# ultravideo/kvazaar

Measured on AMD Instinct MI355X. Metric: CTUs/s (all-intra ultrafast hot path), higher is better.
Workload: dtype u8/i16 (f64 RD costs); 1 GPU; 1920x1080 yuv420p 8-bit all-intra ultrafast CTU pass (kvz_hip_intra_frames), QP 22; ctus_per_frame=510, distinct_frames=8, wpp=True, parallelism=frames sharded over 1 GPU(s), no data-path collective

## Files before the change

### include/kvz_hip_dev.h

```cpp
#ifndef KVZ_HIP_DEV_H_
#define KVZ_HIP_DEV_H_

#include "kvz_hip_types.h"

#ifdef __cplusplus
extern "C" {
#endif

void *kvz_hip_dev_alloc(size_t bytes);
void  kvz_hip_dev_free(void *p);
void  kvz_hip_dev_upload(void *dev_dst, const void *host_src, size_t bytes);
void  kvz_hip_dev_download(void *host_dst, const void *dev_src, size_t bytes);
void  kvz_hip_dev_sync(void);
void  kvz_hip_dev_copy(void *dev_dst, const void *dev_src, size_t bytes);
void  kvz_hip_dev_timer_start(void);
float kvz_hip_dev_timer_stop(void);

int  kvz_hip_dev_sad_nxn(int n, const uint8_t *a, const uint8_t *b, int count, uint32_t *out);
int  kvz_hip_dev_satd_nxn(int n, const uint8_t *a, const uint8_t *b, int count, uint32_t *out);

int  kvz_hip_dev_transform(int kind, const int16_t *in, int16_t *tmp, int16_t *out, int count, int use_matrix_cores);

int  kvz_hip_dev_angular_pred(int log2_width, int mode, const uint8_t *ref_above, const uint8_t *ref_left, int count, uint8_t *out);

int  kvz_hip_dev_intra_select(int log2w, int nblk, const uint32_t *raw, const int8_t *preds, const double *mode_bits, int count, int32_t *winner);

int  kvz_hip_dev_cu8_units(int count, int from_coeffs, const int16_t *in, const int32_t *qp, int16_t *levels, int16_t *dequant, int16_t *resid);

int  kvz_hip_dev_satd8_blocks(const uint8_t *a, const uint8_t *b, int count, uint32_t *out);

int  kvz_hip_dev_rough_rows(int log2w, const uint8_t *top, const uint8_t *left, int count, uint8_t *out);

void kvz_hip_dev_deblock_frames(uint8_t *frames, int width, int height, int n_frames, const uint8_t *cu_depth, int qp, int beta_offset_div2,
                                int tc_offset_div2);

typedef struct kvz_hip_cu_dbk {
  uint8_t type;
  uint8_t depth, tr_depth, part_size;
  uint8_t cbf_y;
  uint8_t mv_dir;
  int8_t  mv_ref[2];
  int16_t ref_id[2];
  int16_t mv[2][2];
} kvz_hip_cu_dbk;
void kvz_hip_dev_deblock_frames_inter(uint8_t *frames, int width, int height, int n_frames, const kvz_hip_cu_dbk *info, int qp, int beta_offset_div2,
                                      int tc_offset_div2, int slice_is_b);
// ... 131 lines not shown
```

### kvazaar_amd/csrc/kvz_ctu.hpp

```cpp
#pragma once
#include <type_traits>
#include "../../include/kvz_hip_types.h"
#include "kvz_ops.hpp"
#include "kvz_rdoq.hpp"
#include "kvz_recon.hpp"
#include "kvz_residual.hpp"
#include "kvz_select.hpp"

namespace kvz {

#define KVZ_CTU_THREADS 128
#ifdef KVZ_HOSTSIM
#define KVZ_FOR_THREADS(tid) for (int tid = 0; tid < KVZ_CTU_THREADS; ++tid)
#ifdef KVZ_HOSTSIM_COUNT_SYNCS
static unsigned long long g_kvz_syncs;
#define KVZ_SYNC() (++g_kvz_syncs)
#else
#define KVZ_SYNC()
#endif
#define KVZ_LDS_ADD(p, v) (*(p) += (v))
#else
#define KVZ_FOR_THREADS(tid) for (int tid = (threadIdx.x + lane_rot) & (KVZ_CTU_THREADS - 1), once_ = 1; once_; once_ = 0)
#define KVZ_SYNC() __syncthreads()
#define KVZ_LDS_ADD(p, v) atomicAdd((p), (v))
// ... 62 lines not shown
  const unsigned t = __builtin_amdgcn_alignbit(x, x, 16);
  Pk16 sw, r;
  __builtin_memcpy(&sw, &t, 4);
  r = a * pk_make(1, -1) + sw;
  unsigned rr;
  __builtin_memcpy(&rr, &r, 4);
  return __builtin_amdgcn_sad_u16(rr, 0x80008000u, acc);
}
#define KVZ_PK_BIAS pk_make(-32768, 0)
#endif

#ifndef KVZ_HOSTSIM
}
#include "kvz_mfma.hpp"
namespace kvz {
#endif

#define KVZ_PROF_PU_AT (2 * KVZ_P_COUNT + 16)
#define KVZ_PROF_W32_AT (4 * KVZ_P_COUNT + 16)
#define KVZ_PROF_WORDS (6 * KVZ_P_COUNT + 16)
enum { KVZ_P_INIT = 0, KVZ_P_REFS, KVZ_P_PRED35, KVZ_P_SATD, KVZ_P_SELECT, KVZ_P_RPRED, KVZ_P_FDCT, KVZ_P_QUANT, KVZ_P_IDCT, KVZ_P_RECON,
       KVZ_P_COST, KVZ_P_COPY, KVZ_P_FINISH, KVZ_P_MISC, KVZ_P_COEFFBITS, KVZ_P_RDOQ, KVZ_P_COUNT };
#if defined(KVZ_CTU_PROFILE) && !defined(KVZ_HOSTSIM)
#define KVZ_PROF(cat) prof_mark(cat)
#define KVZ_PROF_SYNC(cat) do { KVZ_SYNC(); prof_mark(cat); } while (0)
#else
#define KVZ_PROF(cat)
#define KVZ_PROF_SYNC(cat)
#endif

// ... 750 lines not shown
        s->ref[c][side][k] = have ? base[off] : (u8)128;
        if (c) s->ref[2][side][k] = have ? base[off + dv] : (u8)128;
      }
    }
    KVZ_SYNC();
    KVZ_FOR_THREADS(tid) {
      if (luma) {
        const int n = 2 * (1 << log2w_y) + 1;
        for (int i = tid; i < 2 * n; i += KVZ_CTU_THREADS) {
          const int side = i >= n, k = side ? i - n : i;
          s->fref[side][k] = luma_filtered_ref(&s->ref[0][0][0], n, i);
        }
      }
      const int c = mover_lane(tid) - (KVZ_CTU_THREADS - 3);
      if (c >= 0 && ((c == 0 && luma) || (c > 0 && chroma))) {
        const int l2 = c ? log2w_c : log2w_y, w = 1 << l2;
#ifdef KVZ_HOSTSIM
        s->dcval[c] = (u8)dc_value(l2, s->ref[c][0], s->ref[c][1]);
#else
        u32 sum = 0;
        for (int i = 0; i < w; i += 4) {
          u32 a, b;
          __builtin_memcpy(&a, &s->ref[c][0][1 + i], 4);
          __builtin_memcpy(&b, &s->ref[c][1][1 + i], 4);
          sum = __builtin_amdgcn_sad_u8(a, 0u, sum);
          sum = __builtin_amdgcn_sad_u8(b, 0u, sum);
        }
        s->dcval[c] = (u8)((sum + w) >> (l2 + 1));
#endif
      }
    }
    KVZ_SYNC();
    KVZ_PROF(KVZ_P_REFS);
  }

  KVZ_DEV u8 predict_pixel(int log2w, int mode, int c, int x, int y) const
  {
    const int w = 1 << log2w;
    const u8 *top = s->ref[c][0], *left = s->ref[c][1];
    if (c == 0 && luma_reads_filtered(log2w, mode)) { top = s->fref[0]; left = s->fref[1]; }
    if (mode == 0) return planar_pixel(log2w, x, y, top, left);
    if (mode == 1) {
      const int dc = s->dcval[c];
// ... 26 lines not shown
      const u8 *pa = a + r * as, *pb = b + r * bs;
      int d[8];
      for (int x = 0; x < 8; x++) d[x] = (int)pa[x] - (int)pb[x];
      int u0, u1, u2, u3;
      if (col & 4) { u0 = d[0] - d[4]; u1 = d[1] - d[5]; u2 = d[2] - d[6]; u3 = d[3] - d[7]; }
      else { u0 = d[0] + d[4]; u1 = d[1] + d[5]; u2 = d[2] + d[6]; u3 = d[3] + d[7]; }
      const int v0 = (col & 2) ? u0 - u2 : u0 + u2, v1 = (col & 2) ? u1 - u3 : u1 + u3;
      t[r] = (col & 1) ? v0 - v1 : v0 + v1;
    }
    KVZ_HAD8(t[0], t[1], t[2], t[3], t[4], t[5], t[6], t[7]);
    u32 sum = 0;
    for (int r = 0; r < 8; r++) sum += (u32)iabs(t[r]);
    return sum;
  }

#ifndef KVZ_HOSTSIM
  KVZ_DEV static Pk16 as_pk16(U16x2 v) { Pk16 r; __builtin_memcpy(&r, &v, 4); return r; }
  KVZ_DEV static void widen8(const u8 *p, U16x2 out[4])
  {
    unsigned w[2];
    __builtin_memcpy(w, p, 8);
    out[0] = widen(0, w[0], 0x0c010c00u); out[1] = widen(0, w[0], 0x0c030c02u); out[2] = widen(0, w[1], 0x0c010c00u); out[3] = widen(0, w[1], 0x0c030c02u);
  }
#endif
  template <bool PAIR>
  KVZ_DEV u32 angular_block_satd(int log2w, int mode, int bx, int by, int xl, int yl, int half) const
  {
    const int w = 1 << log2w;
    const bool big = S32 && log2w == 5;
    const bool flat = mode < 2;
    const bool vertical = mode >= 18 || flat;
    const int disp = s->mode_disp[mode];
    const int p0 = vertical ? bx : by, q0 = vertical ? by : bx;
    const u8 *mr;
    if (disp < 0) mr = big ? mref32() + (mode - 11) * KVZ_MREF32_STRIDE + KVZ_MREF32_ORG : s->mref[mode - 11] + KVZ_MREF_ORG;
    else {
      const bool filt = imin(iabs(mode - 26), iabs(mode - 10)) > (log2w == 3 ? 7 : (log2w == 4 ? 1 : 0));
      mr = filt ? s->fref[vertical ? 0 : 1] : s->ref[0][vertical ? 0 : 1];
    }
// ... 81 lines not shown
#ifndef KVZ_HOSTSIM
      return sum;
#endif
    }
    return 2 * sum;
  }

#ifndef KVZ_HOSTSIM
  KVZ_DEV u32 angular_group_satd(const SatdWalsh &wm, const dev_int4 rows[2], const dev_int4 o[2]) const
  {
    dev_int4 p[2];
    satd_rows_predict(&s->ref[0][0][0], rows, p);
    return satd8_group_mfma(wm, p, o);
  }

  KVZ_DEV u32 flat_block_satd8(int log2w, int mode, int bx, int by, int xl, int yl, int lane) const
  {
    const int w = 1 << log2w, r = lane & 7, y = by + r;
    U16x2 o[4], v[4];
    widen8(org_at(0, xl + bx, yl + y), o);
    if (mode == 0) {
      const u8 *top = s->fref[0], *left = s->fref[1];
      const int tr = top[w + 1], bl = left[w + 1], l = left[y + 1];
      U16x2 tp[4];
      widen8(top + bx + 1, tp);
      const U16x2 dl = splat16(tr - l), wy = splat16(w - 1 - y), hb = splat16((w - 1) * l + tr + (y + 1) * bl + w);
#pragma unroll
      for (int j = 0; j < 4; j++) {
        U16x2 xs;
        xs.x = (unsigned short)(bx + 2 * j); xs.y = (unsigned short)(bx + 2 * j + 1);
        v[j] = (xs * dl + (tp[j] * wy + hb)) >> (unsigned short)(log2w + 1);
      }
    } else if (mode == 1) {
      const u8 *top = s->ref[0][0], *left = s->ref[0][1];
      const int dc = s->dcval[0];
      U16x2 tp[4];
      widen8(top + bx + 1, tp);
#pragma unroll
      for (int j = 0; j < 4; j++) v[j] = y == 0 ? (U16x2)((tp[j] + splat16(3 * dc + 2)) >> (unsigned short)2) : splat16(dc);
      if (bx == 0) v[0].x = (unsigned short)(y == 0 ? (left[1] + 2 * dc + top[1] + 2) >> 2 : (left[y + 1] + 3 * dc + 2) >> 2);
    } else {
      widen8(s->fref[0] + bx + y + 2, v);
    }
    Pk16 d[4];
#pragma unroll
    for (int j = 0; j < 4; j++) d[j] = as_pk16(v[j] - o[j]);
    if (r == 0) d[0] = pk_add(d[0], KVZ_PK_BIAS);
    {
      const Pk16 a0 = pk_add(d[0], d[2]), a1 = pk_add(d[1], d[3]), a2 = pk_sub(d[0], d[2]), a3 = pk_sub(d[1], d[3]);
      d[0] = pk_add(a0, a1); d[1] = pk_sub(a0, a1); d[2] = pk_add(a2, a3); d[3] = pk_sub(a2, a3);
    }
#define KVZ_FLAT8_STAGE(ctrl, bit)                                                                          \
    {                                                                                                       \
      const Pk16 sgn = pk_make((lane & (bit)) ? -1 : 1, (lane & (bit)) ? -1 : 1);                           \
      _Pragma("unroll") for (int j = 0; j < 4; j++) {                                                       \
        int mine;                                                                                           \
        __builtin_memcpy(&mine, &d[j], 4);                                                                  \
        const int theirs = __builtin_amdgcn_update_dpp(0, mine, ctrl, 0xF, 0xF, true);                       \
        Pk16 ot;                                                                                            \
        __builtin_memcpy(&ot, &theirs, 4);                                                                  \
        d[j] = ot * sgn + d[j];                                                                             \
      }                                                                                                     \
    }
    KVZ_FLAT8_STAGE(0x141 , 4)
    KVZ_FLAT8_STAGE(0x4E , 2)
    KVZ_FLAT8_STAGE(0xB1 , 1)
#undef KVZ_FLAT8_STAGE
    u32 sum = pk_abs2_biased(d[3], pk_abs2_biased(d[2], pk_abs2_biased(d[1], pk_abs2_biased(d[0], 0))));
    sum += (u32)__builtin_amdgcn_update_dpp(0, (int)sum, 0xB1, 0xF, 0xF, true);
    sum += (u32)__builtin_amdgcn_update_dpp(0, (int)sum, 0x4E, 0xF, 0xF, true);
    sum += (u32)__builtin_amdgcn_update_dpp(0, (int)sum, 0x141, 0xF, 0xF, true);
    return sum;
  }
#endif

  template <int L2>
  KVZ_DEV void build_mref(int tid, const u32 *pre = nullptr)
  {
    constexpr int W = 1 << L2, NQ = 2 * W + 2, N = (15 * NQ + KVZ_CTU_THREADS - 1) / KVZ_CTU_THREADS;
    u8 vals[N];
    if constexpr (L2 != 5) {
      static_assert(N * KVZ_CTU_THREADS <= 512, "Tables::mref_tab rows");
      u32 e[N];
      for (int k = 0; k < N; k++) e[k] = pre ? pre[k] : tb->mref_tab[L2 - 3][tid + k * KVZ_CTU_THREADS];
      mref_copy<N>(&s->ref[0][0][0], e);
      return;
    }
    for (int k = 0; k < N; k++) {
// ... 77 lines not shown
  {
    const int log2w = 6 - depth, w = 1 << log2w, xl = x - cx, yl = y - cy, nblk = (w >> 3) * (w >> 3);
#ifndef KVZ_HOSTSIM
    u32 mref_pre[4] = { 0, 0, 0, 0 };
    if (!(S32 && log2w == 5)) {
      const u32 *row = tb->mref_tab[log2w - 3] + ((threadIdx.x + lane_rot) & (KVZ_CTU_THREADS - 1));
      for (int k = 0; k < 4; k++) mref_pre[k] = row[k * KVZ_CTU_THREADS];
    }
    dev_int4 rows_pre[2][2] = {};
    {
      const int t = (threadIdx.x + lane_rot) & (KVZ_CTU_THREADS - 1);
      if (log2w == 4 || (log2w == 3 && t < 64)) {
        const dev_int4 *row = reinterpret_cast<const dev_int4 *>(tb->satd_rows[log2w == 4 ? 1 + 2 * (t >> 6) : 0][t & 63]);
        rows_pre[0][0] = row[0]; rows_pre[0][1] = row[1];
        if (log2w == 4) { rows_pre[1][0] = row[2 * 64]; rows_pre[1][1] = row[2 * 64 + 1]; }
      }
    }
#endif
    build_refs(lv, x, y, log2w, depth == 3 ? 2 : log2w - 1, true, true, first);
    if (S32 && log2w == 5) {
      KVZ_FOR_THREADS(tid) {
        if constexpr (S32) build_mref<5>(tid);
        u8 *ot = org_t32();
        for (int e = tid; e < 1024; e += KVZ_CTU_THREADS) ot[e] = *org_at(0, xl + (e >> 5), yl + (e & 31));
        for (int v = tid; v < 35; v += KVZ_CTU_THREADS) s->satd_raw[v][0] = 0;
        if (tid == KVZ_CTU_THREADS - 1) {
          int left, above;
          neighbour_pair(lv, x, y, &left, &above);
          mpm_candidates(y, left, above, s->preds);
        }
// ... 48 lines not shown
      }
#else
      if (log2w == 4 || tid < 64) {
        const int lane = tid & 63;
        const SatdWalsh wm = satd8_walsh(tb, lane);
        dev_int4 o[2];
        satd_rows_source(&s->ref[0][0][0], org_at(0, xl, yl), rows_pre[0], o);
        const int p = (log2w == 4 ? 64 * (tid >> 6) : 0) + (lane & 31), mode = 2 + (p >> lb), b = p & (nblk - 1);
        const u32 v0 = angular_group_satd(wm, rows_pre[0], o);
        if (lane < 32) s->satd_raw[mode][b] = v0;
        if (log2w == 4) {
          const u32 v1 = angular_group_satd(wm, rows_pre[1], o);
          if (lane < 32) s->satd_raw[mode + 8][b] = v1;
        }
      }
      {
        const int t = KVZ_CTU_THREADS - 1 - tid;
        if (t < 24 * nblk) {
          const int mb = t >> 3, mi = mb >> lb, mode = mi == 0 ? 34 : mi - 1, b = mb & (nblk - 1), bx = (b & ((w >> 3) - 1)) * 8, by = (b >> (log2w - 3)) * 8;
          const u32 v = flat_block_satd8(log2w, mode, bx, by, xl, yl, tid);
          if ((tid & 7) == 0) s->satd_raw[mode][b] = v;
        }
      }
#endif
    }
    }
    KVZ_SYNC();
    KVZ_PROF(KVZ_P_SATD);
    KVZ_FOR_THREADS(tid) {
      if (tid >= kHookThread && tid < kHookThread + kCostEntries) cu_cost_prepare(lv, x, y, depth, tid - kHookThread);
      const int final_mode = replay_selection(tid, log2w, nblk);
      if (final_mode >= 0) {
        if (tid == 0) s->best_mode = final_mode;
#ifdef KVZ_HOSTSIM
        const int holders = 1;
#else
// ... 1839 lines not shown
```

### kvazaar_amd/csrc/kvz_dev.hpp

```cpp
#pragma once
#include <hip/hip_runtime.h>

#include <functional>
#include <mutex>
#include <chrono>
#include <vector>

#include "../../include/kvz_hip_dev.h"
#include "kvz_mfma.hpp"
#include "kvz_ops.hpp"
#include "kvz_sao.hpp"
#include "kvz_entropy.hpp"
#include "kvz_select.hpp"
#include "kvz_recon.hpp"
#include "kvz_tables.hpp"

namespace kvz {

__device__ __forceinline__ u32 load_u32_any(const u8 *p) { u32 v; __builtin_memcpy(&v, p, 4); return v; }
template <int G> __device__ __forceinline__ u32 group_sum(u32 v)
{
  for (int off = G / 2; off > 0; off >>= 1) v += __shfl_down(v, off, G);
  return v;
}
// ... 317 lines not shown
    const int g = L2 == 4 ? 2 * (tid >> 6) + j : 0, pr = 32 * g + (lane & 31), mode = 2 + (pr >> LB), b = pr & (NBLK - 1);
    const dev_int4 *row = reinterpret_cast<const dev_int4 *>(tb->satd_rows[L2 == 4 ? 1 + g : 0][lane]);
    const dev_int4 e[2] = { row[0], row[1] };
    dev_int4 p[2];
    satd_rows_predict(ref0, e, p);
    u8 *o = out + ((cu * 32 + (mode - 2)) * NBLK + b) * 64;
#pragma unroll
    for (int i = 0; i < 4; i++)
#pragma unroll
      for (int x = 0; x < 8; x++) {
        const int r = 4 * (lane >> 5) + i;
        const u8 v = (u8)(((u32)p[i >> 1][2 * (i & 1) + (x >> 2)] >> (8 * (x & 3))) ^ 0x80);
        o[mode >= 18 ? 8 * r + x : 8 * x + r] = v;
      }
  }
}

template <int L2> __global__ void __launch_bounds__(256) dev_angular_kernel(const u8 *above, const u8 *left, const int count, const int mode, u8 *out)
{
  constexpr int W = 1 << L2, NG = kAngularGroupsPerLane, GPB = W * W / 4, BLOCKS = 256 * NG / GPB, RS = 2 * W + 1, ES = (2 * W + 1 + 8 + 3) & ~3;
  constexpr int RAW = (BLOCKS * RS + 3 + 3) / 4 + 2;
  __shared__ u32 s_raw[2][RAW];
  __shared__ alignas(8) u8 s_ext[BLOCKS][ES];
  __shared__ u32 s_tile[BLOCKS * W * W / 4];
  const int disp_tab[9] = { 0, 2, 5, 9, 13, 17, 21, 26, 32 };
  const int inv_tab[9] = { 0, 4096, 1638, 910, 630, 482, 390, 315, 256 };
  const bool vertical = mode >= 18;
  const int mode_disp = vertical ? mode - 26 : 10 - mode, ad = iabs(mode_disp);
  const int disp = mode_disp < 0 ? -disp_tab[ad] : disp_tab[ad], inv = inv_tab[ad];
  const long blk0 = (long)blockIdx.x * BLOCKS;
// ... 873 lines not shown
}

int kvz_hip_dev_cu8_units(int count, int from_coeffs, const int16_t *in, const int32_t *qp, int16_t *levels, int16_t *dequant, int16_t *resid)
{
  if (count < 0 || (from_coeffs != 0 && from_coeffs != 1)) { fprintf(stderr, "kvz_hip_dev_cu8_units: count=%d from_coeffs=%d\n", count, from_coeffs); return -1; }
  if (count == 0) return 0;
  KVZ_DEV_LAUNCH(kvz::dev_cu8_units_kernel, ((long)count + 1) / 2 * 256, in, qp, count, from_coeffs, kvz::device_tables(), levels, dequant, resid);
  return 0;
}

int kvz_hip_dev_rough_rows(int log2w, const uint8_t *top, const uint8_t *left, int count, uint8_t *out)
{
  if (count < 0 || (log2w != 3 && log2w != 4)) { fprintf(stderr, "kvz_hip_dev_rough_rows: log2w=%d count=%d\n", log2w, count); return -1; }
  if (log2w == 3) KVZ_DEV_LAUNCH(kvz::dev_rough_rows_kernel<3>, ((long)count + 1) / 2 * 256, kvz::device_tables(), top, left, count, out);
  else KVZ_DEV_LAUNCH(kvz::dev_rough_rows_kernel<4>, ((long)count + 1) / 2 * 256, kvz::device_tables(), top, left, count, out);
  return 0;
}

int kvz_hip_dev_satd8_blocks(const uint8_t *a, const uint8_t *b, int count, uint32_t *out)
{
  if (count < 0) { fprintf(stderr, "kvz_hip_dev_satd8_blocks: count=%d\n", count); return -1; }
  KVZ_DEV_LAUNCH(kvz::dev_satd8_blocks_kernel, ((long)count + 31) / 32 * 64, kvz::device_tables(), a, b, count, out);
  return 0;
}

void kvz_hip_dev_deblock_frames(uint8_t *frames, int width, int height, int n_frames, const uint8_t *cu_depth, int qp, int beta_offset_div2,
                                int tc_offset_div2)
{
  kvz::deblock_frames_on(be().stream, frames, width, height, n_frames, cu_depth, qp, beta_offset_div2, tc_offset_div2);
}
// ... 1035 lines not shown
```

### kvazaar_amd/csrc/kvz_mfma.hpp

```cpp
#pragma once
#include <hip/hip_runtime.h>

#include "kvz_ops.hpp"

namespace kvz {

typedef int dev_int4 __attribute__((ext_vector_type(4)));
typedef int dev_int16 __attribute__((ext_vector_type(16)));

__device__ __forceinline__ void dev_byte_planes(int v0, int v1, int v2, int v3, u32 &lo, u32 &hi)
{
  const u32 t01 = __builtin_amdgcn_perm((u32)v1, (u32)v0, 0x05010400u), t23 = __builtin_amdgcn_perm((u32)v3, (u32)v2, 0x05010400u);
  lo = __builtin_amdgcn_perm(t23, t01, 0x05040100u) ^ 0x80808080u;
  hi = __builtin_amdgcn_perm(t23, t01, 0x07060302u);
}

template <int N> struct DevMma;
template <> struct DevMma<16> {
  static constexpr int NREG = 4;
  static __device__ __forceinline__ int idx(int lane) { return lane & 15; }
  static __device__ __forceinline__ int row(int lane, int r) { return 4 * (lane >> 4) + r; }
  static __device__ __forceinline__ int k0(int lane, int) { return 4 * (lane >> 4); }
  static constexpr int STEPS = 1;
};
// ... 181 lines not shown
  }
}
__device__ __forceinline__ void satd_rows_source(const u8 *ref0, const u8 *cu_org, const dev_int4 e[2], dev_int4 o[2])
{
  const u8 *base = ((unsigned)e[0][1] >> 16 & kSatdSrcVertical) ? cu_org : ref0;
#pragma unroll
  for (int i = 0; i < 4; i++) {
    const unsigned src = (unsigned)e[i >> 1][2 * (i & 1) + 1] >> 16 & (kSatdSrcVertical - 1);
    unsigned ow[2];
    __builtin_memcpy(ow, __builtin_assume_aligned(base + src, 8), 8);
    o[i >> 1][2 * (i & 1)] = (int)(ow[0] ^ 0x80808080u);
    o[i >> 1][2 * (i & 1) + 1] = (int)(ow[1] ^ 0x80808080u);
  }
}

__device__ __forceinline__ void dev_satd8_blocks_wave(const Tables *tb, const u8 *a, const u8 *bsrc, int count, u32 *out, int group, int lane)
{
  const long blk = 32l * group + (lane & 31);
  const bool live = blk < count;
  dev_int4 p[2] = {}, o[2] = {};
  if (live) {
    const dev_int4 *pa = reinterpret_cast<const dev_int4 *>(a + 64 * blk + 32 * (lane >> 5)), *po = reinterpret_cast<const dev_int4 *>(bsrc + 64 * blk + 32 * (lane >> 5));
    p[0] = pa[0]; p[1] = pa[1]; o[0] = po[0]; o[1] = po[1];
  }
#pragma unroll
  for (int q = 0; q < 2; q++) { p[q] ^= (int)0x80808080u; o[q] ^= (int)0x80808080u; }
  const u32 v = satd8_group_mfma(satd8_walsh(tb, lane), p, o);
  if (live && lane < 32) out[blk] = v;
}

// ... 2 lines not shown
```

### kvazaar_amd/csrc/kvz_ops.hpp

```cpp
#pragma once
#include <stdint.h>

#ifdef KVZ_HOSTSIM
#define KVZ_DEV inline
#define KVZ_ATOMIC_ADD(p, v) (*(p) += (v))
#else
#include <hip/hip_runtime.h>
#define KVZ_DEV __device__ __forceinline__
#define KVZ_ATOMIC_ADD(p, v) atomicAdd((p), (v))
#endif

namespace kvz {

typedef uint8_t u8;
typedef int16_t i16;
typedef uint16_t u16;
typedef uint32_t u32;
typedef int32_t i32;

#ifdef KVZ_HOSTSIM
#define KVZ_HD inline
#else
#define KVZ_HD __host__ __device__ __forceinline__
#endif
// ... 34 lines not shown
  alignas(16) i32 dct_sum[2][2][32];
  alignas(16) int8_t bd_i8[3][2][16 * 16];
  alignas(16) i32 bd_sum[3][2][16];
  u32 small_pairs[3][2][8][4];
  u32 pairs16[2][16][8];
  u32 scan[3][4][1024];
  u8 avail_top[16][16], avail_left[16][16];
  u8 ctx_next[2][128];
  u32 mref_tab[2][512];
  u8 diag8[64];
  u32 entropy_bits[128];
  int8_t luma_filter[4][8];
  int8_t chroma_filter[8][4];
  alignas(16) u32 satd_walsh[64][8];
  alignas(16) u32 satd_rows[5][64][8];
};

struct SatdRow { unsigned window, edge, src; int df; bool vertical; };
KVZ_HD SatdRow satd_row_of(u32 w0, u32 w1)
{
  SatdRow r;
  r.window = w0 & 0xffff; r.edge = w0 >> 16; r.df = (int)(w1 & 0xffff) >> 3; r.vertical = (w1 >> 16 & kSatdSrcVertical) != 0; r.src = w1 >> 16 & (kSatdSrcVertical - 1);
  return r;
}
KVZ_HD void satd_row_walk(const u8 *ref0, u32 w0, u32 w1, u8 out[8])
{
  const SatdRow r = satd_row_of(w0, w1);
  const u8 *m = ref0 + r.window;
  for (int k = 0; k < 8; k++) out[k] = (u8)(((32 - r.df) * m[k] + r.df * m[k + 1] + 16) >> 5);
  out[0] ^= ref0[r.edge];
}
KVZ_HD u8 satd_edge_byte(const u8 *ref0, int log2w, int i)
{
  const int o = i >> log2w, q = i & ((1 << log2w) - 1);
  const u8 *side = ref0 + kMrefRefRow * (1 - o);
  const int main1 = ref0[kMrefRefRow * o + 1];
  return (u8)(iclip(0, 255, main1 + (((int)side[q + 1] - (int)side[0]) >> 1)) ^ main1);
}
template <int N> KVZ_DEV void mref_copy(u8 *ref0, const u32 e[N])
{
  u8 vals[N];
  for (int k = 0; k < N; k++) vals[k] = ref0[e[k] & 0xffff];
  for (int k = 0; k < N; k++) ref0[kMrefExtended + (e[k] >> 16)] = vals[k];
}
KVZ_HD u8 luma_filtered_ref(const u8 *ref0, int n, int i)
{
  const int side = i >= n, k = side ? i - n : i;
  const u8 *r = ref0 + kMrefRefRow * side;
  if (k == 0) return (u8)((ref0[kMrefRefRow + 1] + 2 * ref0[kMrefRefRow] + ref0[1] + 2) / 4);
  if (k == n - 1) return r[k];
  return (u8)((r[k - 1] + 2 * r[k] + r[k + 1] + 2) / 4);
}
// ... 417 lines not shown
{
  const int w = 1 << log2w;
  const int hor = (w - 1 - x) * left[y + 1] + (x + 1) * top[w + 1];
  const int ver = (w - 1 - y) * top[x + 1] + (y + 1) * left[w + 1];
  return (u8)((ver + hor + w) >> (log2w + 1));
}

KVZ_DEV int dc_value(int log2w, const u8 *top, const u8 *left)
{
  const int w = 1 << log2w;
  int sum = 0;
  for (int i = 0; i < w; i++) sum += top[i + 1] + left[i + 1];
  return (u8)((sum + w) >> (log2w + 1));
}

KVZ_DEV u8 filtered_dc_pixel(int dc, int x, int y, const u8 *top, const u8 *left)
{
  if (x == 0 && y == 0) return (u8)((left[1] + 2 * dc + top[1] + 2) / 4);
  if (y == 0) return (u8)((top[x + 1] + 3 * dc + 2) / 4);
  if (x == 0) return (u8)((left[y + 1] + 3 * dc + 2) / 4);
  return (u8)dc;
}

struct IntraPredOp {
  int kind, log2w; const int8_t *modes ; const u8 *above; const u8 *left; long ref_bstride; u8 *dst;
  KVZ_DEV void operator()(int item) const
  {
    const int w = 1 << log2w, blk = item >> (2 * log2w), e = item & (w * w - 1), y = e >> log2w, x = e & (w - 1);
    const u8 *t = above + blk * ref_bstride, *l = left + blk * ref_bstride;
    u8 v;
// ... 151 lines not shown
```

### kvazaar_amd/csrc/kvz_tables.hpp

```cpp
#pragma once
#include <assert.h>
#include <string.h>

#include "kvz_recon.hpp"
#include "kvz_syntax.hpp"

namespace kvz {

inline int dct32_entry(int k, int n)
{
  static const int mag[32] = { 64, 90, 90, 90, 89, 88, 87, 85, 83, 82, 80, 78, 75, 73, 70, 67,
                               64, 61, 57, 54, 50, 46, 43, 38, 36, 31, 25, 22, 18, 13, 9,  4 };
  if (k == 0) return 64;
  const int m = (k * (2 * n + 1)) % 128;
  if (m < 32) return mag[m];
  if (m < 64) return -mag[64 - m];
  if (m < 96) return -mag[m - 64];
  return mag[128 - m];
}

inline void scan_pattern(int type, int size, int *xs, int *ys)
{
  int n = 0;
  if (type == 0) {
// ... 104 lines not shown
        for (int i = 0; i < 4; i++) {
          static const int disp_tab[9] = { 0, 2, 5, 9, 13, 17, 21, 26, 32 };
          const int w = 1 << l2, lb = 2 * (l2 - 3), p = 32 * g + (lane & 31), mode = 2 + (p >> lb), b = p & ((1 << lb) - 1);
          const int bx = (b & ((w >> 3) - 1)) * 8, by = (b >> (l2 - 3)) * 8, r = 4 * (lane >> 5) + i;
          const int vertical = mode >= 18, md = vertical ? mode - 26 : 10 - mode, disp = md < 0 ? -disp_tab[-md] : disp_tab[md];
          const int p0 = vertical ? bx : by, q0 = vertical ? by : bx, qa = q0 + r + 1, delta = qa * disp, df = delta & 31, di = (delta - df) / 32;
          const unsigned row = disp < 0 ? kMrefExtended + kMrefStride * (mode - 11) : (luma_reads_filtered(l2, mode) ? kMrefFiltered : 0u) + kMrefRefRow * (vertical ? 0 : 1);
          const int at = (disp < 0 ? (int)kMrefOrg : 0) + p0 + 1 + di;
          assert(at >= 0 && at + (int)kSatdWindow <= (int)(disp < 0 ? kMrefStride : kMrefRefRow));
          const unsigned edge = disp == 0 && p0 == 0 ? kSatdEdge + 1 + (vertical ? 0 : w) + qa - 1 : kSatdEdge;
          const unsigned src = vertical ? kSatdSrcVertical | (unsigned)((by + r) * 32 + bx) : kSatdSrcT + (unsigned)((bx + r) * w + by);
          u32 *e = t->satd_rows[l2 == 3 ? 0 : 1 + g][lane] + 2 * i;
          e[0] = (row + (unsigned)at) | edge << 16;
          e[1] = (unsigned)(8 * df) | src << 16;
        }
  for (int lane = 0; lane < 64; lane++)
    for (int q = 0; q < 4; q++) { t->satd_walsh[lane][q] = satd_walsh_word(lane, q); t->satd_walsh[lane][4 + q] = satd_walsh_word(lane, q) ^ 0xfefefefeu; }
  static const i16 dst4[16] = { 29, 55, 74, 84, 74, 74, 0, -74, 84, -29, -74, 55, 55, -84, 74, -29 };
  memcpy(t->dst4, dst4, sizeof dst4);
  for (int kind = 0; kind < 3; kind++) {
    const int n = kind == 1 ? 8 : 4;
    const i16 *m = kind == 2 ? t->dst4 : t->dct[kind == 1 ? 1 : 0];
    for (int g = 0; g < 16 / n; g++)
      for (int k = 0; k < n; k++)
        for (int j = 0; j < n; j++) {
          t->bd_i8[kind][0][(g * n + k) * 16 + g * n + j] = (int8_t)m[k * n + j];
          t->bd_i8[kind][1][(g * n + j) * 16 + g * n + k] = (int8_t)m[k * n + j];
          t->bd_sum[kind][0][g * n + k] += m[k * n + j];
          t->bd_sum[kind][1][g * n + j] += m[k * n + j];
        }
// ... 103 lines not shown
```

### kvazaar_amd/dev.py

```python
import ctypes as C

import numpy as np

TRANSFORM_KINDS = {"dct4": 0, "dct8": 1, "dct16": 2, "dct32": 3, "dst4": 4, "idct4": 5, "idct8": 6, "idct16": 7, "idct32": 8, "idst4": 9}
TRANSFORM_SIZE = {0: 4, 1: 8, 2: 16, 3: 32, 4: 4, 5: 4, 6: 8, 7: 16, 8: 32, 9: 4}


class Dev:
    def __init__(self, cdll):
        self.lib = l = cdll
        vp, sz, ci = C.c_void_p, C.c_size_t, C.c_int
        l.kvz_hip_dev_alloc.restype = vp; l.kvz_hip_dev_alloc.argtypes = [sz]
        l.kvz_hip_dev_free.restype = None; l.kvz_hip_dev_free.argtypes = [vp]
        l.kvz_hip_dev_upload.restype = None; l.kvz_hip_dev_upload.argtypes = [vp, vp, sz]
        l.kvz_hip_dev_download.restype = None; l.kvz_hip_dev_download.argtypes = [vp, vp, sz]
        l.kvz_hip_dev_sync.restype = None; l.kvz_hip_dev_sync.argtypes = []
        l.kvz_hip_dev_timer_start.restype = None; l.kvz_hip_dev_timer_start.argtypes = []
        l.kvz_hip_dev_timer_stop.restype = C.c_float; l.kvz_hip_dev_timer_stop.argtypes = []
        for f in (l.kvz_hip_dev_sad_nxn, l.kvz_hip_dev_satd_nxn):
            f.restype = None; f.argtypes = [ci, vp, vp, ci, vp]
        l.kvz_hip_dev_transform.restype = None; l.kvz_hip_dev_transform.argtypes = [ci, vp, vp, vp, ci, ci]
        l.kvz_hip_dev_angular_pred.restype = None; l.kvz_hip_dev_angular_pred.argtypes = [ci, ci, vp, vp, ci, vp]
        l.kvz_hip_dev_intra_select.restype = ci; l.kvz_hip_dev_intra_select.argtypes = [ci, ci, vp, vp, vp, ci, vp]
        l.kvz_hip_dev_cu8_units.restype = ci; l.kvz_hip_dev_cu8_units.argtypes = [ci, ci, vp, vp, vp, vp, vp]
        l.kvz_hip_dev_satd8_blocks.restype = ci; l.kvz_hip_dev_satd8_blocks.argtypes = [vp, vp, ci, vp]
        if hasattr(l, "kvz_hip_dev_rough_rows"):
            l.kvz_hip_dev_rough_rows.restype = ci; l.kvz_hip_dev_rough_rows.argtypes = [ci, vp, vp, ci, vp]

    def put(self, a):
        a = np.ascontiguousarray(a)
        p = self.lib.kvz_hip_dev_alloc(a.nbytes)
        self.lib.kvz_hip_dev_upload(p, a.ctypes.data, a.nbytes)
        return p

    def copy_in(self, p, a):
        a = np.ascontiguousarray(a)
        self.lib.kvz_hip_dev_upload(p, a.ctypes.data, a.nbytes)

    def empty(self, nbytes):
        return self.lib.kvz_hip_dev_alloc(nbytes)

    def get(self, p, shape, dtype):
# ... 8 lines not shown
```

Measured before the change: 3.585 million CTUs/s.

## Table-drive flat-mode SATD lanes and pack two rows per lane for 16x16

Replaces the per-lane flat_block_satd8 (planar/DC/mode-34 SATD) with a table-driven flat_task_satd. Each lane's predictor coefficients, source offset, output slot and butterfly signs are precomputed into Tables::flat_lanes, and 16x16 blocks handle two rows per lane, so fewer lanes do the work and the per-lane branching goes away. The 8x8 lane descriptor is prefetched into rows_pre alongside the angular rows. A KVZ_FLAT16 switch, which defaults to 0, keeps the old one-row-per-lane path for 16x16. The change also adds a standalone rough_flat kernel and API for testing, and costs extra table memory and register pressure.

New measurement: 3.585 million CTUs/s, median of 3. About the same (+0.0%).

```diff
diff --git a/include/kvz_hip_dev.h b/include/kvz_hip_dev.h
--- a/include/kvz_hip_dev.h
+++ b/include/kvz_hip_dev.h
@@ -30,6 +30,8 @@
 int  kvz_hip_dev_satd8_blocks(const uint8_t *a, const uint8_t *b, int count, uint32_t *out);
 
 int  kvz_hip_dev_rough_rows(int log2w, const uint8_t *top, const uint8_t *left, int count, uint8_t *out);
+
+int  kvz_hip_dev_rough_flat(int log2w, const uint8_t *top, const uint8_t *left, const uint8_t *src, int count, uint8_t *pred_out, uint32_t *satd_out);
 
 void kvz_hip_dev_deblock_frames(uint8_t *frames, int width, int height, int n_frames, const uint8_t *cu_depth, int qp, int beta_offset_div2,
                                 int tc_offset_div2);
diff --git a/kvazaar_amd/csrc/kvz_ctu.hpp b/kvazaar_amd/csrc/kvz_ctu.hpp
--- a/kvazaar_amd/csrc/kvz_ctu.hpp
+++ b/kvazaar_amd/csrc/kvz_ctu.hpp
@@ -100,6 +100,71 @@
 }
 #include "kvz_mfma.hpp"
 namespace kvz {
+
+KVZ_DEV Pk16 as_pk16(U16x2 v) { Pk16 r; __builtin_memcpy(&r, &v, 4); return r; }
+template <int L2> struct FlatLaneRows { FlatLane first; FlatSecond second; };
+template <int L2> KVZ_DEV FlatLaneRows<L2> flat_lane_rows(const Tables *tb, int t)
+{
+  FlatLaneRows<L2> f = {};
+  const dev_int4 *a = reinterpret_cast<const dev_int4 *>(tb->flat_lanes[t]) + 4 * (L2 - 3);
+  const dev_int4 q[4] = { a[0], a[1], a[2], a[3] };
+  __builtin_memcpy(&f.first, q, sizeof f.first);
+  if constexpr (L2 == 4) {
+    const dev_int4 p[2] = { a[4], a[5] };
+    __builtin_memcpy(&f.second, p, sizeof f.second);
+  }
+  return f;
+}
+template <int CTRL, int N> KVZ_DEV void flat_exchange(Pk16 *d, u32 sign)
+{
+  Pk16 sgn;
+  __builtin_memcpy(&sgn, &sign, 4);
+#pragma unroll
+  for (int j = 0; j < N; j++) {
+    int mine;
+    __builtin_memcpy(&mine, &d[j], 4);
+    const int theirs = __builtin_amdgcn_update_dpp(0, mine, CTRL, 0xF, 0xF, true);
+    Pk16 ot;
+    __builtin_memcpy(&ot, &theirs, 4);
+    d[j] = ot * sgn + d[j];
+  }
+}
+template <int L2, int NR = FlatTasks<L2>::kRows> KVZ_DEV u32 flat_task_satd(const u8 *ref0, int dc, const u8 *src, const FlatLaneRows<L2> &f, bool first_row, U16x2 (*pred)[4] = nullptr)
+{
+  const int bx = L2 == 3 ? 0 : (int)f.first.src & 31;
+  Pk16 d[NR][4];
+#pragma unroll
+  for (int i = 0; i < NR; i++) {
+    U16x2 v[4], o[4];
+    flat_row_predict<L2>(ref0, i ? flat_second_row(f.first.row, f.second) : f.first.row, bx, dc, v);
+    widen8(static_cast<const u8 *>(__builtin_assume_aligned(src + f.first.src + 4 * 32 * i, 8)), o);
+#pragma unroll
+    for (int j = 0; j < 4; j++) {
+      if (pred) pred[i][j] = v[j];
+      d[i][j] = as_pk16(v[j] - o[j]);
+    }
+  }
+  if (first_row) d[0][0] = pk_add(d[0][0], KVZ_PK_BIAS);
+#pragma unroll
+  for (int i = 0; i < NR; i++) {
+    const Pk16 a0 = pk_add(d[i][0], d[i][2]), a1 = pk_add(d[i][1], d[i][3]), a2 = pk_sub(d[i][0], d[i][2]), a3 = pk_sub(d[i][1], d[i][3]);
+    d[i][0] = pk_add(a0, a1); d[i][1] = pk_sub(a0, a1); d[i][2] = pk_add(a2, a3); d[i][3] = pk_sub(a2, a3);
+  }
+  Pk16 *e = &d[0][0];
+  if constexpr (NR == 2) {
+#pragma unroll
+    for (int j = 0; j < 4; j++) { const Pk16 lo = d[0][j], hi = d[1][j]; d[0][j] = pk_add(lo, hi); d[1][j] = pk_sub(lo, hi); }
+  } else flat_exchange<0x141 , 4>(e, f.first.sign[2]);
+  flat_exchange<0x4E , 4 * NR>(e, f.first.sign[1]);
+  flat_exchange<0xB1 , 4 * NR>(e, f.first.sign[0]);
+  u32 sum = 0;
+#pragma unroll
+  for (int j = 0; j < 4 * NR; j++) sum = pk_abs2_biased(e[j], sum);
+  sum += (u32)__builtin_amdgcn_update_dpp(0, (int)sum, 0xB1, 0xF, 0xF, true);
+  sum += (u32)__builtin_amdgcn_update_dpp(0, (int)sum, 0x4E, 0xF, 0xF, true);
+  if constexpr (NR == 1) sum += (u32)__builtin_amdgcn_update_dpp(0, (int)sum, 0x141, 0xF, 0xF, true);
+  return sum;
+}
 #endif
 
 #define KVZ_PROF_PU_AT (2 * KVZ_P_COUNT + 16)
@@ -880,19 +945,11 @@
       }
       const int c = mover_lane(tid) - (KVZ_CTU_THREADS - 3);
       if (c >= 0 && ((c == 0 && luma) || (c > 0 && chroma))) {
-        const int l2 = c ? log2w_c : log2w_y, w = 1 << l2;
+        const int l2 = c ? log2w_c : log2w_y;
 #ifdef KVZ_HOSTSIM
         s->dcval[c] = (u8)dc_value(l2, s->ref[c][0], s->ref[c][1]);
 #else
-        u32 sum = 0;
-        for (int i = 0; i < w; i += 4) {
-          u32 a, b;
-          __builtin_memcpy(&a, &s->ref[c][0][1 + i], 4);
-          __builtin_memcpy(&b, &s->ref[c][1][1 + i], 4);
-          sum = __builtin_amdgcn_sad_u8(a, 0u, sum);
-          sum = __builtin_amdgcn_sad_u8(b, 0u, sum);
-        }
-        s->dcval[c] = (u8)((sum + w) >> (l2 + 1));
+        s->dcval[c] = (u8)dc_value_sad(l2, s->ref[c][0], s->ref[c][1]);
 #endif
       }
     }
@@ -949,15 +1006,6 @@
     return sum;
   }
 
-#ifndef KVZ_HOSTSIM
-  KVZ_DEV static Pk16 as_pk16(U16x2 v) { Pk16 r; __builtin_memcpy(&r, &v, 4); return r; }
-  KVZ_DEV static void widen8(const u8 *p, U16x2 out[4])
-  {
-    unsigned w[2];
-    __builtin_memcpy(w, p, 8);
-    out[0] = widen(0, w[0], 0x0c010c00u); out[1] = widen(0, w[0], 0x0c030c02u); out[2] = widen(0, w[1], 0x0c010c00u); out[3] = widen(0, w[1], 0x0c030c02u);
-  }
-#endif
   template <bool PAIR>
   KVZ_DEV u32 angular_block_satd(int log2w, int mode, int bx, int by, int xl, int yl, int half) const
   {
@@ -1069,64 +1117,6 @@
     return satd8_group_mfma(wm, p, o);
   }
 
-  KVZ_DEV u32 flat_block_satd8(int log2w, int mode, int bx, int by, int xl, int yl, int lane) const
-  {
-    const int w = 1 << log2w, r = lane & 7, y = by + r;
-    U16x2 o[4], v[4];
-    widen8(org_at(0, xl + bx, yl + y), o);
-    if (mode == 0) {
-      const u8 *top = s->fref[0], *left = s->fref[1];
-      const int tr = top[w + 1], bl = left[w + 1], l = left[y + 1];
-      U16x2 tp[4];
-      widen8(top + bx + 1, tp);
-      const U16x2 dl = splat16(tr - l), wy = splat16(w - 1 - y), hb = splat16((w - 1) * l + tr + (y + 1) * bl + w);
-#pragma unroll
-      for (int j = 0; j < 4; j++) {
-        U16x2 xs;
-        xs.x = (unsigned short)(bx + 2 * j); xs.y = (unsigned short)(bx + 2 * j + 1);
-        v[j] = (xs * dl + (tp[j] * wy + hb)) >> (unsigned short)(log2w + 1);
-      }
-    } else if (mode == 1) {
-      const u8 *top = s->ref[0][0], *left = s->ref[0][1];
-      const int dc = s->dcval[0];
-      U16x2 tp[4];
-      widen8(top + bx + 1, tp);
-#pragma unroll
-      for (int j = 0; j < 4; j++) v[j] = y == 0 ? (U16x2)((tp[j] + splat16(3 * dc + 2)) >> (unsigned short)2) : splat16(dc);
-      if (bx == 0) v[0].x = (unsigned short)(y == 0 ? (left[1] + 2 * dc + top[1] + 2) >> 2 : (left[y + 1] + 3 * dc + 2) >> 2);
-    } else {
-      widen8(s->fref[0] + bx + y + 2, v);
-    }
-    Pk16 d[4];
-#pragma unroll
-    for (int j = 0; j < 4; j++) d[j] = as_pk16(v[j] - o[j]);
-    if (r == 0) d[0] = pk_add(d[0], KVZ_PK_BIAS);
-    {
-      const Pk16 a0 = pk_add(d[0], d[2]), a1 = pk_add(d[1], d[3]), a2 = pk_sub(d[0], d[2]), a3 = pk_sub(d[1], d[3]);
-      d[0] = pk_add(a0, a1); d[1] = pk_sub(a0, a1); d[2] = pk_add(a2, a3); d[3] = pk_sub(a2, a3);
-    }
-#define KVZ_FLAT8_STAGE(ctrl, bit)                                                                          \
-    {                                                                                                       \
-      const Pk16 sgn = pk_make((lane & (bit)) ? -1 : 1, (lane & (bit)) ? -1 : 1);                           \
-      _Pragma("unroll") for (int j = 0; j < 4; j++) {                                                       \
-        int mine;                                                                                           \
-        __builtin_memcpy(&mine, &d[j], 4);                                                                  \
-        const int theirs = __builtin_amdgcn_update_dpp(0, mine, ctrl, 0xF, 0xF, true);                       \
-        Pk16 ot;                                                                                            \
-        __builtin_memcpy(&ot, &theirs, 4);                                                                  \
-        d[j] = ot * sgn + d[j];                                                                             \
-      }                                                                                                     \
-    }
-    KVZ_FLAT8_STAGE(0x141 , 4)
-    KVZ_FLAT8_STAGE(0x4E , 2)
-    KVZ_FLAT8_STAGE(0xB1 , 1)
-#undef KVZ_FLAT8_STAGE
-    u32 sum = pk_abs2_biased(d[3], pk_abs2_biased(d[2], pk_abs2_biased(d[1], pk_abs2_biased(d[0], 0))));
-    sum += (u32)__builtin_amdgcn_update_dpp(0, (int)sum, 0xB1, 0xF, 0xF, true);
-    sum += (u32)__builtin_amdgcn_update_dpp(0, (int)sum, 0x4E, 0xF, 0xF, true);
-    sum += (u32)__builtin_amdgcn_update_dpp(0, (int)sum, 0x141, 0xF, 0xF, true);
-    return sum;
-  }
 #endif
 
   template <int L2>
@@ -1234,6 +1224,9 @@
         const dev_int4 *row = reinterpret_cast<const dev_int4 *>(tb->satd_rows[log2w == 4 ? 1 + 2 * (t >> 6) : 0][t & 63]);
         rows_pre[0][0] = row[0]; rows_pre[0][1] = row[1];
         if (log2w == 4) { rows_pre[1][0] = row[2 * 64]; rows_pre[1][1] = row[2 * 64 + 1]; }
+      } else if (log2w == 3) {
+        const dev_int4 *row = reinterpret_cast<const dev_int4 *>(tb->flat_lanes[t & 63]);
+        rows_pre[0][0] = row[0]; rows_pre[0][1] = row[1]; rows_pre[1][0] = row[2]; rows_pre[1][1] = row[3];
       }
     }
 #endif
@@ -1312,12 +1305,40 @@
           if (lane < 32) s->satd_raw[mode + 8][b] = v1;
         }
       }
-      {
+#ifndef KVZ_FLAT16
+#define KVZ_FLAT16 0
+#endif
+#if KVZ_FLAT16 == 0
+      if (log2w == 4) {
         const int t = KVZ_CTU_THREADS - 1 - tid;
-        if (t < 24 * nblk) {
-          const int mb = t >> 3, mi = mb >> lb, mode = mi == 0 ? 34 : mi - 1, b = mb & (nblk - 1), bx = (b & ((w >> 3) - 1)) * 8, by = (b >> (log2w - 3)) * 8;
-          const u32 v = flat_block_satd8(log2w, mode, bx, by, xl, yl, tid);
-          if ((tid & 7) == 0) s->satd_raw[mode][b] = v;
+        if (t < 96) {
+          const int pr = t >> 3, kind = pr >> 2, b = pr & 3, bx = (b & 1) * 8, by = (b >> 1) * 8, r = tid & 7;
+          FlatLaneRows<4> f = {};
+          f.first.row = flat_row_of(4, kind, bx, by + r);
+          f.first.src = (u32)((by + r) * 32 + bx);
+          for (int k = 0; k < 3; k++) f.first.sign[k] = (u32)(((tid << (31 - k)) >> 31) | 0x00010001);
+          const u32 v = flat_task_satd<4, 1>(&s->ref[0][0][0], s->dcval[0], org_at(0, xl, yl), f, r == 0);
+          if (r == 0) s->satd_raw[kind ? kind - 1 : 34][b] = v;
+        }
+      } else
+#endif
+      if (tid >= 64) {
+        const int t = tid - 64;
+        const u8 *ref0 = &s->ref[0][0][0], *src = org_at(0, xl, yl);
+        const int dc = s->dcval[0];
+        u32 *raw = &s->satd_raw[0][0];
+        static_assert(sizeof s->satd_raw[0] == 16 && sizeof rows_pre == sizeof(FlatLane), "FlatLane::out; an 8x8 CU's FlatLane travels in rows_pre");
+        if (log2w == 3) {
+          if (t < FlatTasks<3>::kLanes) {
+            FlatLaneRows<3> f = {};
+            __builtin_memcpy(&f.first, rows_pre, sizeof f.first);
+            const u32 v = flat_task_satd<3>(ref0, dc, src, f, (t & 7) == 0);
+            if ((t & 7) == 0) raw[f.first.out] = v;
+          }
+        } else if (t < FlatTasks<4>::kLanes) {
+          const FlatLaneRows<4> f = flat_lane_rows<4>(tb, t);
+          const u32 v = flat_task_satd<4>(ref0, dc, src, f, (t & 3) == 0);
+          if ((t & 3) == 0) raw[f.first.out] = v;
         }
       }
 #endif
diff --git a/kvazaar_amd/csrc/kvz_dev.hpp b/kvazaar_amd/csrc/kvz_dev.hpp
--- a/kvazaar_amd/csrc/kvz_dev.hpp
+++ b/kvazaar_amd/csrc/kvz_dev.hpp
@@ -355,6 +355,40 @@
         o[mode >= 18 ? 8 * r + x : 8 * x + r] = v;
       }
   }
+}
+
+template <int L2> __global__ void __launch_bounds__(256) dev_rough_flat_kernel(const Tables *tb, const u8 *top, const u8 *left, const u8 *src, const int count, u8 *pred_out, u32 *satd_out)
+{
+  constexpr int W = 1 << L2, N = 2 * W + 1, NBLK = 1 << (2 * (L2 - 3)), NR = FlatTasks<L2>::kRows, REFS = (kMrefFiltered + 2 * kMrefRefRow + 15) & ~15u;
+  static_assert(2 * N <= 128 && FlatTasks<L2>::kLanes <= 64 && W * W / 8 <= 128, "a lane per reference sample, per eight source samples; the tasks of one wavefront");
+  __shared__ alignas(16) u8 lds[2][REFS + 16 * 32];
+  __shared__ int dcv[2];
+  const int half = threadIdx.x >> 7, tid = threadIdx.x & 127;
+  const long cu = 2l * blockIdx.x + half;
+  const bool live = cu < count;
+  u8 *ref0 = lds[half];
+  const int side = tid >= N, k = side ? tid - N : tid;
+  if (live && tid < 2 * N) ref0[kMrefRefRow * side + k] = (side ? left : top)[cu * N + k];
+  if (live && tid < W * W / 8) *reinterpret_cast<uint2 *>(ref0 + REFS + 32 * (tid / (W / 8)) + 8 * (tid % (W / 8))) = *reinterpret_cast<const uint2 *>(src + cu * W * W + 8 * tid);
+  __syncthreads();
+  if (live && tid < 2 * N) ref0[kMrefFiltered + kMrefRefRow * side + k] = luma_filtered_ref(ref0, N, tid);
+  if (live && tid == 127) dcv[half] = dc_value_sad(L2, ref0, ref0 + kMrefRefRow);
+  __syncthreads();
+  const int t = tid - 64;
+  if (!live || t < 0 || t >= FlatTasks<L2>::kLanes) return;
+  const FlatTasks<L2> task(t);
+  const FlatLaneRows<L2> f = flat_lane_rows<L2>(tb, t);
+  U16x2 pred[NR][4];
+  const u32 sum = flat_task_satd<L2>(ref0, dcv[half], ref0 + REFS, f, task.row == 0, pred);
+  const long pair = (cu * 3 + (task.kind + 2) % 3) * NBLK + task.block;
+#pragma unroll
+  for (int i = 0; i < NR; i++) {
+    unsigned vw[4];
+    __builtin_memcpy(vw, pred[i], 16);
+    const uint2 row = { __builtin_amdgcn_perm(vw[1], vw[0], 0x06040200u), __builtin_amdgcn_perm(vw[3], vw[2], 0x06040200u) };
+    *reinterpret_cast<uint2 *>(pred_out + pair * 64 + 8 * (task.row + 4 * i)) = row;
+  }
+  if (task.row == 0) satd_out[pair] = sum;
 }
 
 template <int L2> __global__ void __launch_bounds__(256) dev_angular_kernel(const u8 *above, const u8 *left, const int count, const int mode, u8 *out)
@@ -1258,6 +1292,14 @@
   if (count < 0 || (log2w != 3 && log2w != 4)) { fprintf(stderr, "kvz_hip_dev_rough_rows: log2w=%d count=%d\n", log2w, count); return -1; }
   if (log2w == 3) KVZ_DEV_LAUNCH(kvz::dev_rough_rows_kernel<3>, ((long)count + 1) / 2 * 256, kvz::device_tables(), top, left, count, out);
   else KVZ_DEV_LAUNCH(kvz::dev_rough_rows_kernel<4>, ((long)count + 1) / 2 * 256, kvz::device_tables(), top, left, count, out);
+  return 0;
+}
+
+int kvz_hip_dev_rough_flat(int log2w, const uint8_t *top, const uint8_t *left, const uint8_t *src, int count, uint8_t *pred_out, uint32_t *satd_out)
+{
+  if (count < 0 || (log2w != 3 && log2w != 4)) { fprintf(stderr, "kvz_hip_dev_rough_flat: log2w=%d count=%d\n", log2w, count); return -1; }
+  if (log2w == 3) KVZ_DEV_LAUNCH(kvz::dev_rough_flat_kernel<3>, ((long)count + 1) / 2 * 256, kvz::device_tables(), top, left, src, count, pred_out, satd_out);
+  else KVZ_DEV_LAUNCH(kvz::dev_rough_flat_kernel<4>, ((long)count + 1) / 2 * 256, kvz::device_tables(), top, left, src, count, pred_out, satd_out);
   return 0;
 }
 
diff --git a/kvazaar_amd/csrc/kvz_mfma.hpp b/kvazaar_amd/csrc/kvz_mfma.hpp
--- a/kvazaar_amd/csrc/kvz_mfma.hpp
+++ b/kvazaar_amd/csrc/kvz_mfma.hpp
@@ -219,6 +219,31 @@
   }
 }
 
+__device__ __forceinline__ void widen8(const u8 *p, U16x2 out[4])
+{
+  unsigned w[2];
+  __builtin_memcpy(w, p, 8);
+  out[0] = widen(0, w[0], 0x0c010c00u); out[1] = widen(0, w[0], 0x0c030c02u); out[2] = widen(0, w[1], 0x0c010c00u); out[3] = widen(0, w[1], 0x0c030c02u);
+}
+template <int L2> __device__ __forceinline__ void flat_row_predict(const u8 *ref0, const FlatRow &r, int bx, int dc, U16x2 v[4])
+{
+  int bhe[3];
+  flat_row_scalars(ref0, L2, r, bx, dc, bhe);
+  U16x2 t[4];
+  widen8(ref0 + r.window, t);
+  const U16x2 a = splat16(r.a), b = splat16(bhe[0]), s = splat16(r.s);
+  U16x2 h = splat16(bhe[1]), h0 = h;
+  h0.x += (unsigned short)bhe[2];
+#pragma unroll
+  for (int j = 0; j < 4; j++) {
+    U16x2 xs;
+    xs.x = (unsigned short)(2 * j); xs.y = (unsigned short)(2 * j + 1);
+    U16x2 g = xs * b + (j ? h : h0);
+    asm("" : "+v"(g));
+    v[j] = (t[j] * a + g) >> s;
+  }
+}
+
 __device__ __forceinline__ void dev_satd8_blocks_wave(const Tables *tb, const u8 *a, const u8 *bsrc, int count, u32 *out, int group, int lane)
 {
   const long blk = 32l * group + (lane & 31);
diff --git a/kvazaar_amd/csrc/kvz_ops.hpp b/kvazaar_amd/csrc/kvz_ops.hpp
--- a/kvazaar_amd/csrc/kvz_ops.hpp
+++ b/kvazaar_amd/csrc/kvz_ops.hpp
@@ -72,6 +72,7 @@
   int8_t chroma_filter[8][4];
   alignas(16) u32 satd_walsh[64][8];
   alignas(16) u32 satd_rows[5][64][8];
+  alignas(16) u32 flat_lanes[64][40];
 };
 
 struct SatdRow { unsigned window, edge, src; int df; bool vertical; };
@@ -94,6 +95,59 @@
   const u8 *side = ref0 + kMrefRefRow * (1 - o);
   const int main1 = ref0[kMrefRefRow * o + 1];
   return (u8)(iclip(0, 255, main1 + (((int)side[q + 1] - (int)side[0]) >> 1)) ^ main1);
+}
+struct FlatRow { u32 window, side; i32 a, s, kt, kl, ky, kdc, kc, patch, kp; };
+KVZ_HD FlatRow flat_row_of(int log2w, int kind, int bx, int y)
+{
+  const int w = 1 << log2w;
+  const bool planar = kind == 1, dc = kind == 2;
+  FlatRow r;
+  r.window = (dc ? 0u : kMrefFiltered) + (unsigned)(bx + 1 + (kind == 0 ? y + 1 : 0));
+  r.side = (dc ? 0u : kMrefFiltered) + kMrefRefRow + (unsigned)(y + 1);
+  r.a = planar ? w - 1 - y : (dc && y ? 0 : 1);
+  r.s = planar ? log2w + 1 : (dc ? 2 : 0);
+  r.kt = planar ? 1 : 0;
+  r.kl = planar ? w - 1 : 0;
+  r.ky = planar ? y + 1 : 0;
+  r.kdc = dc ? (y ? 4 : 3) : 0;
+  r.kc = planar ? w : (dc && !y ? 2 : 0);
+  r.patch = dc && bx == 0 ? 1 : 0;
+  r.kp = r.patch && y ? 2 : 0;
+  return r;
+}
+KVZ_HD void flat_row_scalars(const u8 *ref0, int log2w, const FlatRow &r, int bx, int dc, int out[3])
+{
+  const int w = 1 << log2w, L = ref0[r.side], tr = ref0[kMrefFiltered + w + 1], bl = ref0[kMrefFiltered + kMrefRefRow + w + 1];
+  out[0] = r.kt * (tr - L);
+  out[1] = r.kl * L + r.kc + r.kt * tr + r.ky * bl + r.kdc * dc + bx * out[0];
+  out[2] = r.patch * (L - dc) + r.kp;
+}
+KVZ_HD void flat_row_walk(const u8 *ref0, int log2w, const FlatRow &r, int bx, int dc, u8 out[8])
+{
+  int bhe[3];
+  flat_row_scalars(ref0, log2w, r, bx, dc, bhe);
+  const u8 *t = ref0 + r.window;
+  for (int j = 0; j < 8; j++) out[j] = (u8)((unsigned short)(t[j] * r.a + j * bhe[0] + bhe[1] + (j == 0 ? bhe[2] : 0)) >> r.s);
+}
+template <int L2> struct FlatTasks {
+  static constexpr int kRows = L2 == 3 ? 1 : 2, kLanesPerPair = 8 / kRows, kPairs = 3 << (2 * (L2 - 3)), kLanes = kPairs * kLanesPerPair;
+  int kind, block, bx, by, row;
+  KVZ_HD explicit FlatTasks(int t)
+  {
+    const int pair = t / kLanesPerPair;
+    kind = pair >> (2 * (L2 - 3)); block = pair & ((1 << (2 * (L2 - 3))) - 1); row = t & (kLanesPerPair - 1);
+    bx = (block & ((1 << (L2 - 3)) - 1)) * 8; by = (block >> (L2 - 3)) * 8;
+  }
+  KVZ_HD int mode() const { return kind ? kind - 1 : 34; }
+};
+struct FlatLane { FlatRow row; u32 src, out, sign[3]; };
+struct FlatSecond { u32 window; i32 a, ky, kdc, kc, kp, pad[2]; };
+static_assert(sizeof(FlatLane) == 64 && sizeof(FlatSecond) == 32, "Tables::flat_lanes");
+KVZ_HD FlatRow flat_second_row(const FlatRow &first, const FlatSecond &f)
+{
+  FlatRow r = first;
+  r.window = f.window; r.side = first.side + 4; r.a = f.a; r.ky = f.ky; r.kdc = f.kdc; r.kc = f.kc; r.kp = f.kp;
+  return r;
 }
 template <int N> KVZ_DEV void mref_copy(u8 *ref0, const u32 e[N])
 {
@@ -541,6 +595,22 @@
   return (u8)((sum + w) >> (log2w + 1));
 }
 
+#ifndef KVZ_HOSTSIM
+KVZ_DEV int dc_value_sad(int log2w, const u8 *top, const u8 *left)
+{
+  const int w = 1 << log2w;
+  u32 sum = 0;
+  for (int i = 0; i < w; i += 4) {
+    u32 a, b;
+    __builtin_memcpy(&a, &top[1 + i], 4);
+    __builtin_memcpy(&b, &left[1 + i], 4);
+    sum = __builtin_amdgcn_sad_u8(a, 0u, sum);
+    sum = __builtin_amdgcn_sad_u8(b, 0u, sum);
+  }
+  return (u8)((sum + w) >> (log2w + 1));
+}
+#endif
+
 KVZ_DEV u8 filtered_dc_pixel(int dc, int x, int y, const u8 *top, const u8 *left)
 {
   if (x == 0 && y == 0) return (u8)((left[1] + 2 * dc + top[1] + 2) / 4);
diff --git a/kvazaar_amd/csrc/kvz_tables.hpp b/kvazaar_amd/csrc/kvz_tables.hpp
--- a/kvazaar_amd/csrc/kvz_tables.hpp
+++ b/kvazaar_amd/csrc/kvz_tables.hpp
@@ -142,6 +142,22 @@
           e[0] = (row + (unsigned)at) | edge << 16;
           e[1] = (unsigned)(8 * df) | src << 16;
         }
+  for (int lane = 0; lane < 64; lane++) {
+    FlatLane f[2];
+    FlatSecond g;
+    const FlatTasks<3> k3(lane < FlatTasks<3>::kLanes ? lane : FlatTasks<3>::kLanes - 1);
+    const FlatTasks<4> k4(lane < FlatTasks<4>::kLanes ? lane : FlatTasks<4>::kLanes - 1);
+    f[0].row = flat_row_of(3, k3.kind, k3.bx, k3.by + k3.row);
+    f[0].src = (u32)((k3.by + k3.row) * 32 + k3.bx); f[0].out = (u32)(4 * k3.mode() + k3.block);
+    f[1].row = flat_row_of(4, k4.kind, k4.bx, k4.by + k4.row);
+    f[1].src = (u32)((k4.by + k4.row) * 32 + k4.bx); f[1].out = (u32)(4 * k4.mode() + k4.block);
+    for (int q = 0; q < 2; q++) for (int b = 0; b < 3; b++) f[q].sign[b] = (lane >> b & 1) ? 0xffffffffu : 0x00010001u;
+    const FlatRow second = flat_row_of(4, k4.kind, k4.bx, k4.by + k4.row + 4);
+    g.window = second.window; g.a = second.a; g.ky = second.ky; g.kdc = second.kdc; g.kc = second.kc; g.kp = second.kp; g.pad[0] = g.pad[1] = 0;
+    const FlatRow again = flat_second_row(f[1].row, g);
+    assert(memcmp(&again, &second, sizeof second) == 0);
+    memcpy(t->flat_lanes[lane], &f[0], sizeof f[0]); memcpy(t->flat_lanes[lane] + 16, &f[1], sizeof f[1]); memcpy(t->flat_lanes[lane] + 32, &g, sizeof g);
+  }
   for (int lane = 0; lane < 64; lane++)
     for (int q = 0; q < 4; q++) { t->satd_walsh[lane][q] = satd_walsh_word(lane, q); t->satd_walsh[lane][4 + q] = satd_walsh_word(lane, q) ^ 0xfefefefeu; }
   static const i16 dst4[16] = { 29, 55, 74, 84, 74, 74, 0, -74, 84, -29, -74, 55, 55, -84, 74, -29 };
diff --git a/kvazaar_amd/dev.py b/kvazaar_amd/dev.py
--- a/kvazaar_amd/dev.py
+++ b/kvazaar_amd/dev.py
@@ -26,6 +26,8 @@
         l.kvz_hip_dev_satd8_blocks.restype = ci; l.kvz_hip_dev_satd8_blocks.argtypes = [vp, vp, ci, vp]
         if hasattr(l, "kvz_hip_dev_rough_rows"):
             l.kvz_hip_dev_rough_rows.restype = ci; l.kvz_hip_dev_rough_rows.argtypes = [ci, vp, vp, ci, vp]
+        if hasattr(l, "kvz_hip_dev_rough_flat"):
+            l.kvz_hip_dev_rough_flat.restype = ci; l.kvz_hip_dev_rough_flat.argtypes = [ci, vp, vp, vp, ci, vp, vp]
 
     def put(self, a):
         a = np.ascontiguousarray(a)
```
